# CederGroupHub/sparse-lm

Measured on AMD Instinct MI355X. Metric: fits/sec over 50-alpha Lasso path at n=100k p=5k, higher is better.
Workload: dtype f64

## Files before the change

sparse-lm_amd/csrc/ws_kernels.hpp:

```cpp
#pragma once
#include <type_traits>
#include <hip/hip_runtime.h>
#include <stdint.h>

#include "tail_kernels.hpp"
#include "newton_kernels.hpp"

namespace slm {

constexpr int WS_KCAP = 512;
constexpr int WS_KLDS = 112;
constexpr int WS_TILES = WS_KCAP / 16;
constexpr int WS_THREADS = 1024;
constexpr int WS_INNER_MAX = 400;
constexpr int WS_BB_ITERS = 14;
constexpr double WS_BB_MAX_STEP = 20.0;
constexpr double WS_INNER_TOL = 0.05;
constexpr int WS_MAX_REPEATS = 6;
constexpr int WS_NEWTON_AFTER = 16;
constexpr int WS_NEWTON_MAX = 256;
constexpr int WS_AFTER_DIRECT = 40;
constexpr double WS_NEWTON_RQ = 0.05;
constexpr int WS_NEWTON_REFUSALS = 4;
constexpr double WS_NEWTON_ENTER = 0.3;
constexpr int WS_NEWTON_RESOLVE = 5;
static_assert(NT_MAXT * NT_B == WS_KCAP, "the direct solve covers a full working set");

struct WsCtl {
  int32_t request;
  int32_t building;
  int32_t valid;
  int32_t K;
  int32_t Kreal;
  int32_t k_new;
  int32_t builds;
  int32_t appends;
  int32_t max_builds;
  int32_t disabled;
  int32_t misses;
  int32_t refined;
  int32_t counter;
  int32_t stale;
  int32_t overflows;
  int32_t sweep_new;
  int32_t sweep_miss;
  int32_t staged;
  int32_t inner_iters;
  int32_t hard;
  int32_t hard_next;
  int32_t newton_steps;
  int32_t newton_fails;
  int32_t newton_nopd;
  int32_t newton_trial[4];
  int32_t newton_ref[4];
  int32_t newton_factors;
  int32_t newton_unknowns;
  unsigned long long nt_ticks[SLM_MAX_LANES][6];
  int32_t nt_factors[SLM_MAX_LANES];
  unsigned long long solve_ticks[5];
  int32_t want_full[SLM_MAX_LANES];
  int32_t iters_hist[32];
  unsigned long long lane_ticks[SLM_MAX_LANES];
  int32_t last_point[SLM_MAX_LANES];
  int32_t repeats[SLM_MAX_LANES];
  int32_t last_cols[SLM_MAX_LANES];
  double Lw[SLM_MAX_LANES];
  int32_t carried;
  int32_t outgrown;
  int32_t served[SLM_MAX_LANES];
  int32_t hard_lane[SLM_MAX_LANES];
};

struct WsArgs {
  WsCtl* ws;
  int32_t* idx;
  int32_t* pos;
  int32_t* gs;
  int32_t* gl;
  double* score;
  double* XW;
  double* part;
  double* Gm;
  double* nt;
  double* Gx;
  const double* X;
  const double* XT;
  int64_t n, ld;
  const double* rw;
  int64_t rw_stride;
  double inv_n[SLM_MAX_LANES];
  int32_t set_of[SLM_MAX_LANES];
  int32_t set_lane[SLM_MAX_LANES];
  int32_t n_sets;
  int32_t nblk;
  const int32_t* owner;
  double theta;
  int32_t lookahead;
  int32_t append_max;
  int32_t k_init;
  int32_t bb_steps;
  int32_t one_solver;
  int32_t miss_factor;
  int32_t miss_div;
  double fill;
  int32_t power_iters;
  int32_t hard_call;
  int32_t keep_full;
};

constexpr int WS_HEAD_WORDS = 24;
static_assert(offsetof(WsCtl, hard_next) / 4 < WS_HEAD_WORDS, "the words the pass kernels decide on");
#define WS_HEAD(hd, field) ((hd)[offsetof(WsCtl, field) / 4])
__device__ __forceinline__ void ws_head_load(const WsCtl* ws, const int* gdone, int32_t* hd) {
  const int tid = threadIdx.x;
  if (tid < WS_HEAD_WORDS) hd[tid] = reinterpret_cast<const int32_t*>(ws)[tid];
  else if (tid == WS_HEAD_WORDS) hd[tid] = gdone ? gdone[0] : 0;
}

static __global__ void ws_ctl_init_kernel(WsCtl* ws, int max_builds) {
  if (threadIdx.x == 0) {
    ws->request = 1;
    ws->max_builds = max_builds;
  }
  if (threadIdx.x < SLM_MAX_LANES) ws->last_point[threadIdx.x] = -1;
}

struct BeginArgs {
  const PathCtl* h_ctl;
  PathCtl* ctl;
  const slm_path_point* h_pts;
  slm_path_point* pts;
  int64_t n_pts;
  int32_t* head;
  int32_t head_words;
  const double* lambda;
  double margin;
  double factor[SLM_MAX_LANES];
  WsCtl* ws;
  int32_t max_builds;
  int32_t n_lanes;
};
static __global__ __launch_bounds__(256) void solve_begin_kernel(SetupArgs s, BeginArgs b) {
  solve_setup_body(s);
  const int64_t stride = (int64_t)gridDim.x * blockDim.x;
  {
    static_assert(sizeof(slm_path_point) == 4 * sizeof(double), "points travel as doubles");
    const double* src = reinterpret_cast<const double*>(b.h_pts);
    double* dst = reinterpret_cast<double*>(b.pts);
    for (int64_t e = (int64_t)blockIdx.x * blockDim.x + threadIdx.x; e < 4 * b.n_pts; e += stride) dst[e] = src[e];
  }
  if (blockIdx.x != 0) return;
  for (int e = threadIdx.x; e < b.head_words; e += 256) b.head[e] = 0;
  {
    static_assert(sizeof(PathCtl) % sizeof(int32_t) == 0, "control blocks travel as words");
    const int32_t* src = reinterpret_cast<const int32_t*>(b.h_ctl);
    int32_t* dst = reinterpret_cast<int32_t*>(b.ctl);
    const int words = b.n_lanes * (int)(sizeof(PathCtl) / sizeof(int32_t));
    for (int e = threadIdx.x; e < words; e += 256) dst[e] = src[e];
  }
  __syncthreads();
  if (b.lambda != nullptr && (int)threadIdx.x < b.n_lanes && threadIdx.x < SLM_MAX_LANES) {
    const int l = threadIdx.x;
    double L0 = b.lambda[0] * b.margin;
    if (L0 <= 0.0) L0 = 1.0;
    const double L = L0 * b.factor[l];
    b.ctl[l].L = L;
    b.ctl[l].ak = 1.25 * L;
    b.ctl[l].Lhat = 0.5 * L0;
  }
  if (b.ws != nullptr) {
    if (threadIdx.x == 0) {
      b.ws->request = 1;
      b.ws->max_builds = b.max_builds;
    }
    if (threadIdx.x < SLM_MAX_LANES) b.ws->last_point[threadIdx.x] = -1;
  }
}

static __global__ __launch_bounds__(256) void ws_ctl_carry_kernel(WsCtl* ws, int max_builds) {
  __shared__ int keep_i[2];
  __shared__ double keep_L[SLM_MAX_LANES];
  if (threadIdx.x == 0) {
    keep_i[0] = ws->K;
    keep_i[1] = ws->Kreal;
  }
  if (threadIdx.x < SLM_MAX_LANES) keep_L[threadIdx.x] = ws->Lw[threadIdx.x];
  __syncthreads();
  int32_t* words = reinterpret_cast<int32_t*>(ws);
  for (int e = threadIdx.x; e < (int)(sizeof(WsCtl) / sizeof(int32_t)); e += 256) words[e] = 0;
  __syncthreads();
  if (threadIdx.x == 0) {
    ws->K = keep_i[0];
    ws->Kreal = keep_i[1];
    ws->valid = 1;
    ws->carried = 1;
    ws->max_builds = max_builds;
  }
  if (threadIdx.x < SLM_MAX_LANES) {
    ws->Lw[threadIdx.x] = keep_L[threadIdx.x];
    ws->last_point[threadIdx.x] = -1;
  }
}

__device__ __forceinline__ int block_excl_scan(int v, int* wave_tot , int* total) {
  const int lane = threadIdx.x & 63, wave = threadIdx.x >> 6;
  int inc = v;
#pragma unroll
  for (int off = 1; off < 64; off <<= 1) {
    const int t = __shfl_up(inc, off, 64);
    if (lane >= off) inc += t;
  }
  __syncthreads();
  if (lane == 63) wave_tot[wave] = inc;
  __syncthreads();
  int base = 0, tot = 0;
#pragma unroll
  for (int w = 0; w < TAIL_WAVES; ++w) {
    const int t = wave_tot[w];
    if (w < wave) base += t;
    tot += t;
  }
  *total = tot;
  return base + inc - v;
}

__device__ __forceinline__ void ws_score_body(TailArgs a, WsArgs w, const int chunk) {
  WsCtl* ws = w.ws;
  const int tid = threadIdx.x;
  __shared__ int32_t hd[WS_HEAD_WORDS + 1];
  __shared__ int lane_np[SLM_MAX_LANES];
  ws_head_load(ws, a.gdone, hd);
  if (tid < SLM_MAX_LANES) lane_np[tid] = tid < a.n_lanes ? a.ctl[tid].n_points : 0;
  __syncthreads();
  if (hd[WS_HEAD_WORDS] != 0 || WS_HEAD(hd, disabled)) return;
  const bool had_w = WS_HEAD(hd, valid) != 0;
  if (!WS_HEAD(hd, request) && !had_w) return;
  if (WS_HEAD(hd, builds) >= WS_HEAD(hd, max_builds) || WS_HEAD(hd, appends) >= 8 * WS_HEAD(hd, max_builds)) return;
  const bool singleton = a.singleton != 0;
  const int nitems = singleton ? a.p : a.G;
  __shared__ int lane_live[SLM_MAX_LANES];
  __shared__ double lane_sa[SLM_MAX_LANES], lane_sb[SLM_MAX_LANES];
  __shared__ int cnt[2];
  if (tid < SLM_MAX_LANES) {
    int live = 0;
    double sa = 0.0, sb = 0.0;
    if (tid < a.n_lanes) {
      const PathCtl* c = a.ctl + tid;
      live = !(c->done || c->idle);
      int path_end = 0;
      for (int l = 0; l < SLM_MAX_LANES; ++l) path_end = max(path_end, lane_np[l]);
      const int end = a.steal ? path_end : c->pt_off + c->n_points;
      int look = min(c->pt_off + c->point + max(w.lookahead, c->stride), end - 1);
      if (c->tail_pt >= 0 && c->point + c->stride >= c->n_points) look = c->pt_off + c->tail_pt;
      const slm_path_point pe = a.pts[look < 0 ? 0 : look];
      sa = pe.sa;
      sb = pe.sb;
    }
    lane_live[tid] = live;
    lane_sa[tid] = sa;
    lane_sb[tid] = sb;
  }
  if (tid == 0) cnt[0] = cnt[1] = 0;
  __syncthreads();

  const double inf = __builtin_huge_val();
  int n_new = 0, n_miss = 0;
  const int gt = chunk * (int)blockDim.x + tid;
  const int it = singleton ? gt : gt >> 4;
  if (singleton) {
    if (it < nitems) {
      double sc = 0.0;
      const int j = it;
      const bool in_w = had_w && w.pos[j] >= 0;
      for (int l0 = 0; l0 < a.n_lanes; l0 += 16) {
        double zp[16], zz[16], aa[16], bb[16], gg[16];
#pragma unroll
        for (int l = 0; l < 16; ++l) {
          const int ll = l0 + l < a.n_lanes ? l0 + l : 0;
          const int64_t off = (int64_t)ll * a.ld;
          zp[l] = a.zprev[off + j];
          zz[l] = a.z[off + j];
          aa[l] = a.a0[off + j];
          bb[l] = a.b0[off + j];
          gg[l] = a.g[(int64_t)ll * (a.ld + 16) + j];
        }
#pragma unroll
        for (int l = 0; l < 16; ++l) {
          if (l0 + l >= a.n_lanes || !lane_live[l0 + l]) continue;
          if (!in_w && had_w && zz[l] != zp[l]) n_miss += 1;
          if (zp[l] != 0.0) {
            sc = inf;
          } else {
            const double thr = lane_sa[l0 + l] * aa[l] + lane_sb[l0 + l] * bb[l];
            sc = fmax(sc, thr > 0.0 ? fabs(gg[l]) / thr : inf);
          }
        }
      }
      if (sc >= w.theta && !in_w) n_new += 1;
      w.score[it] = sc;
    }
  } else {
    static_assert(SLM_MAX_LANES % 16 == 0, "16-thread teams: a thread per (group, lane of a half)");
    const int l16 = tid & 15;
    const bool have = it < nitems;
// ... 190 lines not shown
            ws->stale = 1;
          }
          return;
        }
      }
      append = false;
      thr = w.theta;
    }
  }
  if (!append) {
    count_at(inf, false, &n_sel, nullptr);
    if (n_sel > (double)WS_KCAP) {
      if (tid == 0) {
        ws->overflows += 1;
        ws->outgrown += 1;
        if (had_w) {
          ws->request = 0;
          ws->stale = 1;
        } else {
          ws->request = 1;
          ws->valid = 0;
          if (ws->overflows >= 50) ws->disabled = 1;
        }
      }
      return;
    }
    const double nonzeros = n_sel;
    thr = fit_threshold(w.theta, false, fmax((double)w.k_init, nonzeros), &n_sel);
    for (int j = tid; j < p; j += WS_THREADS) w.pos[j] = -1;
  }
  for (int k = k_old * (append ? 1 : 0) + tid; k < WS_KCAP; k += WS_THREADS) {
    w.idx[k] = -1;
    w.gs[k] = k;
    w.gl[k] = 1;
  }
  __syncthreads();

  unsigned long long pick = 0ull;
  int mine = 0;
  if (cached) {
#pragma unroll
    for (int u = 0; u < 8; ++u) {
      if (c_sc[u] >= thr && !(append && c_inw[u])) {
        pick |= 1ull << u;
        mine += c_sz[u];
      }
    }
  } else {
    for (int it = i0; it < i1 && it - i0 < 64; ++it) {
      if (!(w.score[it] >= thr)) continue;
      if (append && w.pos[singleton ? it : a.order[a.gstart[it]]] >= 0) continue;
      pick |= 1ull << (it - i0);
      mine += singleton ? 1 : a.gstart[it + 1] - a.gstart[it];
    }
  }
  int total = 0;
  int at = (append ? k_old : 0) + block_excl_scan(mine, wave_tot, &total);
  __syncthreads();
  for (int it = i0; it < i1 && it - i0 < 64; ++it) {
    if (!((pick >> (it - i0)) & 1ull)) continue;
    if (singleton) {
      w.idx[at] = it;
      w.pos[it] = at;
      at += 1;
    } else {
      const int k0 = a.gstart[it], len = a.gstart[it + 1] - k0;
      for (int m = 0; m < len; ++m) {
        const int j = a.order[k0 + m];
        w.idx[at + m] = j;
        w.pos[j] = at + m;
        w.gs[at + m] = at;
        w.gl[at + m] = len;
      }
      at += len;
    }
  }
  if (tid == 0) {
    const int Kreal = (append ? k_old : 0) + total;
    ws->Kreal = Kreal;
    ws->K = max(16, (Kreal + 15) & ~15);
    ws->k_new = append ? k_old : 0;
    ws->building = 1;
    ws->valid = 0;
    ws->stale = 0;
    ws->counter = 0;
    if (append) {
      ws->appends += 1;
    } else {
      ws->builds += 1;
      for (int l = 0; l < SLM_MAX_LANES; ++l) ws->Lw[l] = 0.0;
    }
  }
}

static __global__ __launch_bounds__(WS_THREADS) void ws_select_kernel(TailArgs a, WsArgs w) { ws_select_body(a, w); }

static __global__ __launch_bounds__(256) void ws_gather_kernel(WsArgs w) {
  if (!w.ws->building) return;
  const int K = w.ws->K;
  const int k0 = w.ws->k_new + 32 * (int)blockIdx.y;
  if (k0 >= K) return;
  __shared__ double tile[32][33];
  const int tx = threadIdx.x & 31, ty = threadIdx.x >> 5;
  const int64_t row_tiles = (w.n + 31) / 32;
  int jcol[4];
#pragma unroll
  for (int u = 0; u < 4; ++u) {
    const int k = k0 + ty + 8 * u;
    jcol[u] = k < K ? w.idx[k] : -1;
  }
  for (int64_t rt = blockIdx.x; rt < row_tiles; rt += gridDim.x) {
    const int64_t i0 = rt * 32;
    const int64_t i = i0 + tx;
    double v[4];
#pragma unroll
    for (int u = 0; u < 4; ++u) {
      const int j = jcol[u];
      v[u] = (j >= 0 && i < w.n) ? (w.XT ? w.XT[((rt * w.ld + j) << 5) + tx] : w.X[i * w.ld + j]) : 0.0;
    }
    __syncthreads();
#pragma unroll
    for (int u = 0; u < 4; ++u) tile[ty + 8 * u][tx] = v[u];
    __syncthreads();
    for (int ii = ty; ii < 32; ii += 8) {
      const int64_t i = i0 + ii;
      const int k = k0 + tx;
      if (i < w.n && k < K) w.XW[i * WS_KCAP + k] = tile[tx][ii];
    }
  }
}

struct XtyArgs {
  const WsCtl* ws;
  const int32_t* idx;
  const double* XW;
  const double* y;
  double* part;
  double* g;
  double* gprev;
  double* z;
  PathCtl* ctl;
  const int* done;
  int64_t n, ld;
  double inv_n;
  int n_lanes, nblk;
};
static __global__ __launch_bounds__(512) void ws_xty_partial_kernel(XtyArgs a) {
  if (*a.done) return;
  __shared__ double red[8][WS_KCAP];
  __shared__ double red_yy[8];
  const int K = a.ws->K;
  const int lane = threadIdx.x & 63, wave = threadIdx.x >> 6;
  const int64_t rows = (a.n + gridDim.x - 1) / gridDim.x;
  const int64_t i0 = (int64_t)blockIdx.x * rows, i1 = i0 + rows < a.n ? i0 + rows : a.n;
  double acc[WS_KCAP / 64];
#pragma unroll
  for (int c = 0; c < WS_KCAP / 64; ++c) acc[c] = 0.0;
  double yy = 0.0;
  auto rows4 = [&](auto NC) {
    constexpr int C = decltype(NC)::value;
    for (int64_t i = i0 + wave; i < i1; i += 32) {
      double xv[4][C], yv[4];
#pragma unroll
      for (int r = 0; r < 4; ++r) {
        const bool in = i + 8 * r < i1;
        const int64_t ii = in ? i + 8 * r : i;
        yv[r] = in ? a.y[ii] : 0.0;
#pragma unroll
        for (int c = 0; c < C; ++c) {
          const int k = lane + 64 * c;
          xv[r][c] = a.XW[ii * WS_KCAP + (k < K ? k : 64 * c)];
        }
      }
#pragma unroll
      for (int r = 0; r < 4; ++r) {
        yy = __builtin_fma(yv[r], yv[r], yy);
#pragma unroll
        for (int c = 0; c < C; ++c) acc[c] = __builtin_fma(lane + 64 * c < K ? xv[r][c] : 0.0, yv[r], acc[c]);
      }
    }
  };
  switch ((K + 63) >> 6) {
    case 1: rows4(std::integral_constant<int, 1>{}); break;
    case 2: rows4(std::integral_constant<int, 2>{}); break;
    case 3: rows4(std::integral_constant<int, 3>{}); break;
    case 4: rows4(std::integral_constant<int, 4>{}); break;
    case 5: rows4(std::integral_constant<int, 5>{}); break;
    case 6: rows4(std::integral_constant<int, 6>{}); break;
    case 7: rows4(std::integral_constant<int, 7>{}); break;
    default: rows4(std::integral_constant<int, 8>{}); break;
  }
  static_assert(WS_KCAP / 64 == 8, "eight chunks of 64 positions");
#pragma unroll
  for (int c = 0; c < WS_KCAP / 64; ++c) red[wave][lane + 64 * c] = acc[c];
  if (lane == 0) red_yy[wave] = yy;
  __syncthreads();
  double* out = a.part + (int64_t)blockIdx.x * (WS_KCAP + 1);
  const int k = threadIdx.x;
  if (k < K) {
    double sum = 0.0;
#pragma unroll
    for (int w = 0; w < 8; ++w) sum += red[w][k];
    out[k] = sum;
  }
  if (k == WS_KCAP - 1) {
    double sum = 0.0;
#pragma unroll
    for (int w = 0; w < 8; ++w) sum += red_yy[w];
    out[WS_KCAP] = sum;
  }
}
static __global__ __launch_bounds__(512) void ws_xty_apply_kernel(XtyArgs a) {
  if (*a.done) return;
  __shared__ double red[4][128];
  __shared__ double ry[512];
  const int K = a.ws->K;
  const int kl = threadIdx.x & 127, q = threadIdx.x >> 7;
  const int k = (int)blockIdx.x * 128 + kl;
  if ((int)blockIdx.x * 128 >= K) return;
  double s[8] = {0, 0, 0, 0, 0, 0, 0, 0};
  if (k < K) {
    int b = q;
    for (; b + 28 < a.nblk; b += 32) {
#pragma unroll
      for (int u = 0; u < 8; ++u) s[u] += a.part[(int64_t)(b + 4 * u) * (WS_KCAP + 1) + k];
    }
    for (; b < a.nblk; b += 4) s[0] += a.part[(int64_t)b * (WS_KCAP + 1) + k];
  }
  red[q][kl] = ((s[0] + s[1]) + (s[2] + s[3])) + ((s[4] + s[5]) + (s[6] + s[7]));
  if (blockIdx.x == 0) ry[threadIdx.x] = (int)threadIdx.x < a.nblk ? a.part[(int64_t)threadIdx.x * (WS_KCAP + 1) + WS_KCAP] : 0.0;
  __syncthreads();
  if (q == 0 && k < K) {
    const int j = a.idx[k];
    if (j >= 0) {
      const double c = -((red[0][kl] + red[1][kl]) + (red[2][kl] + red[3][kl])) * a.inv_n;
      for (int l = 0; l < a.n_lanes; ++l) {
        a.g[(int64_t)l * (a.ld + 16) + j] = c;
        a.gprev[(int64_t)l * a.ld + j] = c;
        a.z[(int64_t)l * a.ld + j] = 0.0;
      }
    }
  }
  if (blockIdx.x == 0) {
    for (int off = 256; off >= 1; off >>= 1) {
      if ((int)threadIdx.x < off) ry[threadIdx.x] += ry[threadIdx.x + off];
      __syncthreads();
    }
    if (threadIdx.x < (unsigned)a.n_lanes) {
      const int l = threadIdx.x;
      const double loss0 = 0.5 * ry[0] * a.inv_n;
      a.g[(int64_t)l * (a.ld + 16) + a.ld] = loss0;
      a.ctl[l].hist[0] = loss0;
      a.ctl[l].loss_base = loss0;
    }
  }
}

static __global__ __launch_bounds__(256) void ws_block_owner_kernel(const double* rw, int64_t rw_stride, WsArgs w, int32_t* owner) {
  __shared__ int cls[SLM_MAX_LANES];
  __shared__ int red[2][4];
  const int tid = threadIdx.x;
  const int64_t b = blockIdx.x;
  const int64_t base = w.n / w.nblk, rem = w.n % w.nblk;
  const int64_t r0 = b * base + (b < rem ? b : rem);
  const int64_t nrows = base + (b < rem ? 1 : 0);
  for (int st = 0; st < w.n_sets; ++st) {
    const double* v = rw + (int64_t)w.set_lane[st] * rw_stride + r0;
    int zeros = 1, ones = 1;
    for (int64_t i = tid; i < nrows; i += 256) {
      const double x = v[i];
      zeros &= (x == 0.0);
      ones &= (x == 1.0);
    }
    zeros = __all(zeros);
    ones = __all(ones);
    if ((tid & 63) == 0) {
      red[0][tid >> 6] = zeros;
      red[1][tid >> 6] = ones;
    }
    __syncthreads();
    if (tid == 0) {
      const int z = red[0][0] & red[0][1] & red[0][2] & red[0][3], o = red[1][0] & red[1][1] & red[1][2] & red[1][3];
      cls[st] = z ? 0 : (o ? 1 : 2);
    }
    __syncthreads();
  }
  if (tid == 0) {
    int first_ones = -1;
    for (int st = 0; st < w.n_sets; ++st) {
      int o = st;
      if (cls[st] == 0) o = -1;
      else if (cls[st] == 1) {
        if (first_ones < 0) first_ones = st;
        o = first_ones;
      }
      owner[(int64_t)st * w.nblk + b] = o;
    }
  }
}

typedef double ws_d4 __attribute__((ext_vector_type(4)));
constexpr int WS_GRAM_THREADS = 512;
constexpr int WS_GRAM_ZCHUNKS = 4;

static __global__ __launch_bounds__(WS_GRAM_THREADS) void ws_gram_kernel(WsArgs w) {
  if (!w.ws->building) return;
  __shared__ ws_d4 comb[2][16][64];
  const int K = w.ws->K;
  const int tile_lo = w.ws->k_new >> 4;
  const int tid = threadIdx.x, lane = tid & 63;
  const int wave = __builtin_amdgcn_readfirstlane(tid >> 6);
  const int tiles = K >> 4;
  const bool row_split = (tile_lo > 0 || tiles <= 8) && tiles - tile_lo <= 4 * WS_GRAM_ZCHUNKS;
  const int set = blockIdx.y;
  const int64_t b = blockIdx.x;
  if (w.owner != nullptr && w.owner[(int64_t)set * w.nblk + b] != set) return;
  const int64_t base = w.n / w.nblk, rem = w.n % w.nblk;
  const int64_t r0 = b * base + (b < rem ? b : rem);
  const int64_t nrows = base + (b < rem ? 1 : 0);
  const double* rw = w.rw ? w.rw + (int64_t)w.set_lane[set] * w.rw_stride : nullptr;
  const int part = row_split ? (wave >> 1) : 0;
  const int64_t steps = (nrows + 3) >> 2;
  const int64_t s_begin = row_split ? 4 * (steps * part / 4) : 0;
  const int64_t s_end = row_split ? min(nrows, 4 * (steps * (part + 1) / 4)) : nrows;

  for (int slice = 0; slice < 4 * WS_GRAM_ZCHUNKS; ++slice) {
  const int zhi = slice >> 2;
  if (8 * (slice & 3) >= tiles) continue;
  if (row_split ? (tile_lo + 4 * zhi >= tiles) : (zhi >= 2)) continue;
  const int wj = 2 * (slice & 3) + (wave & 1);
  const int ntj = min(4, max(0, tiles - 4 * wj));
  const int ibase = row_split ? tile_lo + 4 * zhi : 4 * (4 * zhi + (wave >> 1));
  const int ti_lo = row_split ? 0 : max(0, tile_lo - ibase);
  const int nti = min(4, max(0, tiles - ibase));
  const bool active = ti_lo < nti && ntj > 0;
  if (!row_split && !active) continue;
  ws_d4 acc[4][4];
#pragma unroll
  for (int ti = 0; ti < 4; ++ti)
#pragma unroll
    for (int tj = 0; tj < 4; ++tj) acc[ti][tj] = ws_d4{0.0, 0.0, 0.0, 0.0};

  const int kk = lane >> 4, c = lane & 15;
  if (active) {
    const int ta_max = WS_TILES - 1;
    const double* rwp = rw ? rw : w.XW;
    const bool has_rw = rw != nullptr;
    auto load = [&](int64_t s, double(&av)[4], double(&bv)[4], double& wgt) {
      const int64_t i = s + kk;
      const bool ok = i < s_end;
      const int64_t row = r0 + (ok ? i : 0);
      const double wv = rwp[has_rw ? row : 0];
      const double* xr = w.XW + row * WS_KCAP + c;
#pragma unroll
      for (int t = 0; t < 4; ++t) {
        av[t] = xr[16 * min(ibase + t, ta_max)];
        bv[t] = xr[16 * min(4 * wj + t, ta_max)];
      }
      wgt = ok ? (has_rw ? wv : 1.0) : 0.0;
    };
    auto mma = [&](const double(&av)[4], const double(&bv)[4], double wgt) {
#pragma unroll
      for (int ti = 0; ti < 4; ++ti) {
        if (ti >= ti_lo && ti < nti) {
          const double a = av[ti] * wgt;
#pragma unroll
          for (int tj = 0; tj < 4; ++tj)
            if (tj < ntj) acc[ti][tj] = __builtin_amdgcn_mfma_f64_16x16x4f64(a, bv[tj], acc[ti][tj], 0, 0, 0);
        }
      }
    };
    double a0[4], b0[4], a1[4], b1[4], a2[4], b2[4], a3[4], b3[4], w0, w1, w2, w3;
    load(s_begin, a0, b0, w0);
    load(s_begin + 4, a1, b1, w1);
    load(s_begin + 8, a2, b2, w2);
    for (int64_t s = s_begin; s < s_end; s += 16) {
      load(s + 12, a3, b3, w3);
      mma(a0, b0, w0);
      load(s + 16, a0, b0, w0);
      mma(a1, b1, w1);
      load(s + 20, a1, b1, w1);
      mma(a2, b2, w2);
      load(s + 24, a2, b2, w2);
      mma(a3, b3, w3);
    }
  }
  if (row_split) {
    for (int round = 0; round < 4; ++round) {
      if (part == round && active) {
#pragma unroll
        for (int ti = 0; ti < 4; ++ti)
#pragma unroll
          for (int tj = 0; tj < 4; ++tj) {
            if (ti < nti && tj < ntj) {
              if (round > 0) acc[ti][tj] += comb[wave & 1][ti * 4 + tj][lane];
              if (round < 3) comb[wave & 1][ti * 4 + tj][lane] = acc[ti][tj];
            }
          }
      }
      __syncthreads();
    }
  }
  if (!row_split || (part == 3 && active)) {
#pragma unroll
  for (int ti = 0; ti < 4; ++ti) {
    if (ti < ti_lo || ti >= nti) continue;
#pragma unroll
    for (int tj = 0; tj < 4; ++tj) {
      if (tj >= ntj) continue;
      const int64_t tile = (int64_t)(ibase + ti) * WS_TILES + (4 * wj + tj);
      double* out = w.part + (((int64_t)set * (WS_TILES * WS_TILES) + tile) * w.nblk + b) * 256;
#pragma unroll
      for (int r = 0; r < 4; ++r) out[(kk + 4 * r) * 16 + c] = acc[ti][tj][r];
    }
  }
  }
  if (row_split) __syncthreads();
  }
}

static __global__ __launch_bounds__(256) void ws_gram_reduce_kernel(WsArgs w) {
  WsCtl* ws = w.ws;
  if (!ws->building) return;
  const int K = ws->K;
  const int row_lo = (ws->k_new >> 4) << 4;
  const int set = blockIdx.y;
  const int tile = blockIdx.x, I = tile / WS_TILES, J = tile % WS_TILES;
  const int tiles = K >> 4, I_lo = row_lo >> 4;
  if (I < I_lo || I >= tiles || J >= tiles) return;
  const int i = 16 * I + (threadIdx.x >> 4), j = 16 * J + (threadIdx.x & 15);
  {
    const double* src = w.part + (((int64_t)set * (WS_TILES * WS_TILES) + tile) * w.nblk) * 256 + threadIdx.x;
    double s4[4] = {0.0, 0.0, 0.0, 0.0};
    int b = 0;
    if (w.owner != nullptr) {
      __shared__ int64_t off_s[512];
      static_assert(sizeof(off_s) >= 8 * 512, "nblk <= 512");
      for (int bb = threadIdx.x; bb < w.nblk; bb += 256) {
        const int o = w.owner[(int64_t)set * w.nblk + bb];
        off_s[bb] = o < 0 ? -1 : (int64_t)(o - set) * (WS_TILES * WS_TILES) * w.nblk * 256;
      }
      __syncthreads();
      for (; b + 32 <= w.nblk; b += 32) {
        double v[32];
#pragma unroll
        for (int u = 0; u < 32; ++u) {
          const int64_t o = off_s[b + u];
          v[u] = o == -1 ? 0.0 : src[(int64_t)(b + u) * 256 + o];
        }
#pragma unroll
        for (int u = 0; u < 32; ++u) s4[u & 3] += v[u];
      }
      for (; b < w.nblk; ++b) {
        const int64_t o = off_s[b];
        s4[b & 3] += o == -1 ? 0.0 : src[(int64_t)b * 256 + o];
      }
    }
    for (; b + 32 <= w.nblk; b += 32) {
      double v[32];
#pragma unroll
      for (int u = 0; u < 32; ++u) v[u] = src[(int64_t)(b + u) * 256];
#pragma unroll
      for (int u = 0; u < 32; ++u) s4[u & 3] += v[u];
    }
    for (; b < w.nblk; ++b) s4[b & 3] += src[(int64_t)b * 256];
    double s = ((s4[0] + s4[1]) + (s4[2] + s4[3])) * w.inv_n[set];
    double* Gs = (w.Gx ? w.Gx : w.Gm) + (int64_t)set * (WS_KCAP * WS_KCAP);
    Gs[i * WS_KCAP + j] = s;
    if (j < row_lo) Gs[j * WS_KCAP + i] = s;
  }
  __threadfence();
  __syncthreads();
  if (threadIdx.x == 0) {
    const int total = (tiles - I_lo) * tiles * (int)gridDim.y;
    if (atomicAdd(&ws->counter, 1) + 1 == total) {
      ws->counter = 0;
      if (w.Gx) {
        ws->staged = 1;
      } else {
        ws->request = 0;
        ws->valid = 1;
        __threadfence();
        ws->building = 0;
      }
    }
  }
}

constexpr int WS_PUBLISH_BLOCKS = 64;
static __global__ __launch_bounds__(256) void ws_publish_kernel(WsArgs w) {
  WsCtl* ws = w.ws;
  if (!ws->building || !ws->staged) return;
  const int K = ws->K;
  const int row_lo = (ws->k_new >> 4) << 4;
  const int set = blockIdx.y;
  for (int i = blockIdx.x; i < K; i += gridDim.x)
    for (int j = threadIdx.x; j < K; j += 256)
      if (i >= row_lo || j >= row_lo) {
        const int64_t at = (int64_t)set * (WS_KCAP * WS_KCAP) + (int64_t)i * WS_KCAP + j;
        w.Gm[at] = w.Gx[at];
      }
  __threadfence();
  __syncthreads();
  if (threadIdx.x == 0) {
    const int total = gridDim.x * gridDim.y;
    if (atomicAdd(&ws->counter, 1) + 1 == total) {
      ws->counter = 0;
      ws->staged = 0;
      ws->request = 0;
      ws->valid = 1;
      __threadfence();
      ws->building = 0;
    }
  }
}

template <int NV>
__device__ __forceinline__ void ws_sum(double (&v)[NV], double (*lds)[TAIL_WAVES], int nwc) {
  const int lane = threadIdx.x & 63;
  const int wave = __builtin_amdgcn_readfirstlane(threadIdx.x >> 6);
  if (wave < nwc) {
#pragma unroll
    for (int k = 0; k < NV; ++k) v[k] = wave_sum_lane63(v[k]);
  }
  __syncthreads();
  if (wave < nwc && lane == 63) {
#pragma unroll
    for (int k = 0; k < NV; ++k) lds[k][wave] = v[k];
  }
  __syncthreads();
  if (nwc == 4) {
#pragma unroll
    for (int k = 0; k < NV; ++k) v[k] = group_sum_all<4>(lds[k][lane & 3]);
  } else {
#pragma unroll
    for (int k = 0; k < NV; ++k) v[k] = group_sum_all<8>(lds[k][lane & 7]);
  }
}

struct WsSolveLds {
  double delta[WS_KCAP];
  double uim[WS_KCAP];
  double part[WS_THREADS];
  double Gl[WS_KLDS * WS_KLDS];
  NtShared nts;
  double nv[WS_KCAP];
  double xsl[WS_KCAP];
  double rgl[WS_KCAP];
  double pbl[WS_KCAP];
  double scale2;
  int nz[WS_KCAP];
  int act[WS_KCAP];
  int rank_of[WS_KCAP];
  int nnz, m;
};

template <bool GROUPED, bool DIRECT>
__device__ __forceinline__ bool ws_refine_lane(TailArgs a, const WsArgs& w, double (*red)[TAIL_WAVES], WsSolveLds& sh) {
  double (&delta)[WS_KCAP] = sh.delta;
  double (&uim)[WS_KCAP] = sh.uim;
  int (&nz)[WS_KCAP] = sh.nz;
  int& nnz_s = sh.nnz;
  double (&part)[WS_THREADS] = sh.part;
  double (&Gl)[WS_KLDS * WS_KLDS] = sh.Gl;
  NtShared& nts = sh.nts;
  double (&nv)[WS_KCAP] = sh.nv;
  int (&act)[WS_KCAP] = sh.act;
  int (&rank_of)[WS_KCAP] = sh.rank_of;
  int& m_s = sh.m;
  double (&xsl)[WS_KCAP] = sh.xsl;
  double (&rgl)[WS_KCAP] = sh.rgl;
  double (&pbl)[WS_KCAP] = sh.pbl;
  double& scale2_s = sh.scale2;
  const int lane_id = blockIdx.x;
  PathCtl* ctl = a.ctl + lane_id;
  WsCtl* ws = w.ws;
  if (!ws->valid || ws->building || ws->disabled) return true;
  const int tid = threadIdx.x;
  const int p = a.p;
  const int K = __builtin_amdgcn_readfirstlane(ws->K);
  const int set = w.set_of[lane_id];
  const double* Gm = w.Gm + (int64_t)set * (WS_KCAP * WS_KCAP);
  {
    const int64_t off = (int64_t)lane_id * a.ld;
    a.beta += off; a.z += off; a.zprev += off; a.gprev += off;
    a.a0 += off; a.b0 += off; a.d0 += off;
    a.pts += ctl->pt_off;
  }
  if (ws->stale) {
    double out[1] = {0.0};
    for (int j = tid; j < p; j += WS_THREADS)
      if (w.pos[j] < 0 && a.z[j] != a.zprev[j]) out[0] += 1.0;
    block_sum<1>(out, red);
    if (out[0] != 0.0) return true;
  }
  const int point_now = ctl->point + ctl->pt_off;
  const int reps = (ws->last_point[lane_id] == point_now && ws->last_cols[lane_id] == ws->Kreal) ? ws->repeats[lane_id] : 0;
  if (reps >= WS_MAX_REPEATS) return true;
  const int hard_now = w.hard_call ? ws->hard : ws->hard_lane[lane_id];
  if (!DIRECT && w.nt != nullptr && hard_now != 0) {
    if (tid == 0) ws->want_full[lane_id] = 1;
    return false;
  }

  unsigned long long tk_s = wall_clock64();
  auto mark = [&](int slot) {
    if (tid == 0 && lane_id == 0) {
      const unsigned long long now = wall_clock64();
      ws->solve_ticks[slot] += now - tk_s;
      tk_s = now;
    }
  };
  const slm_path_point pt = a.pts[ctl->point];
  const int mode = ctl->mode;
  const double tol = ctl->tol;
  const bool group_pen = (pt.sb != 0.0) || (pt.sd != 0.0);
  const bool g_lds = K <= WS_KLDS;
  if (g_lds) {
    for (int e = tid; e < K * K; e += WS_THREADS) {
      const int r = e / K, c = e - r * K;
      Gl[e] = Gm[r * WS_KCAP + c];
    }
  }

  const int tsh = K <= 256 ? 2 : 1;
  const int TPC = 1 << tsh;
  const int KP = WS_THREADS >> tsh;
  const int k = tid & (KP - 1), q = tid >> (10 - tsh);
  static_assert(WS_THREADS == 1024, "q = tid >> (10 - tsh)");
  const int nwc = KP >> 6;
  const int j = k < K ? w.idx[k] : -1;
  const bool live = j >= 0;
  const bool mine = live && q == 0;
  const int jj = live ? j : 0;
  const double z0 = live ? a.zprev[jj] : 0.0;
  const double g0 = live ? a.gprev[jj] : 0.0;
  const double x_start = live ? a.z[jj] : 0.0;
  const double pa = live ? pt.sa * a.a0[jj] : 0.0;
  const int gsk = live ? w.gs[k] : 0, glk = live ? w.gl[k] : 1;
  const int gix = a.singleton ? jj : a.gid[jj];
  const double pb = live ? pt.sb * a.b0[gix] : 0.0;
  const double pd = live ? pt.sd * a.d0[gix] : 0.0;
  __syncthreads();

  auto matvec = [&](double val, bool dense) -> double {
    if (q == 0) delta[k] = (k < K) ? val - z0 : 0.0;
    __syncthreads();
    double acc = 0.0;
    if (g_lds) {
      if (k < K) {
#pragma unroll 4
        for (int c = q; c < K; c += TPC) acc = __builtin_fma(Gl[c * K + k], delta[c], acc);
      }
    } else if (dense) {
      if (k < K) {
        for (int c = __builtin_amdgcn_readfirstlane(q); c < K; c += 16 * TPC) {
          double gv[16];
#pragma unroll
          for (int u = 0; u < 16; ++u) gv[u] = Gm[(c + u * TPC < K ? c + u * TPC : c) * WS_KCAP + k];
#pragma unroll
          for (int u = 0; u < 16; ++u) acc = __builtin_fma(gv[u], c + u * TPC < K ? delta[c + u * TPC] : 0.0, acc);
        }
      }
    } else {
      if (tid < 64) {
        int basep = 0;
        for (int c0 = 0; c0 < K; c0 += 64) {
          const int kk = c0 + tid;
          const bool nzq = kk < K && delta[kk] != 0.0;
          const uint64_t m = __ballot(nzq);
          if (nzq) nz[basep + __popcll(m & ((1ull << tid) - 1ull))] = kk;
          basep += __popcll(m);
        }
        if (tid == 0) nnz_s = basep;
      }
      __syncthreads();
      const int nnz = __builtin_amdgcn_readfirstlane(nnz_s);
      const int qs = __builtin_amdgcn_readfirstlane(q);
      if (k < K) {
        for (int m = qs; m < nnz; m += 12 * TPC) {
          int cc[12];
          double gv[12];
#pragma unroll
          for (int u = 0; u < 12; ++u) cc[u] = __builtin_amdgcn_readfirstlane(nz[m + u * TPC < nnz ? m + u * TPC : m]);
#pragma unroll
          for (int u = 0; u < 12; ++u) gv[u] = Gm[cc[u] * WS_KCAP + k];
#pragma unroll
          for (int u = 0; u < 12; ++u) acc = __builtin_fma(gv[u], m + u * TPC < nnz ? delta[cc[u]] : 0.0, acc);
        }
      }
    }
    part[tid] = acc;
    __syncthreads();
    double tot = part[k];
    for (int qq = 1; qq < TPC; ++qq) tot += part[qq * KP + k];
    return tot;
  };
  auto prox_w = [&](double v, double s) -> double {
    double u = live ? soft(v, s * pa) : 0.0;
    if (group_pen) {
      if (a.singleton) {
        const double nrm = fabs(u);
        const double sc = nrm > 0.0 ? fmax(0.0, 1.0 - s * pb / nrm) : 0.0;
        u *= sc / (1.0 + s * pd);
      } else {
        __syncthreads();
        if (q == 0) uim[k] = u;
        __syncthreads();
        double ss = 0.0;
        for (int m = 0; m < glk; ++m) {
          const double t = uim[gsk + m];
          ss = __builtin_fma(t, t, ss);
        }
        const double nrm = sqrt(ss);
        const double sc = (nrm > 0.0 ? fmax(0.0, 1.0 - s * pb / nrm) : 0.0) / (1.0 + s * pd);
        u *= sc;
      }
    }
    return u;
  };
  auto pen_part = [&](double val) -> double {
    double pv = 0.0;
    if (mine) {
      pv = pa * fabs(val);
      if (group_pen && a.singleton) pv += pb * fabs(val) + 0.5 * pd * val * val;
    }
    if (group_pen && !a.singleton) {
      __syncthreads();
      if (q == 0) uim[k] = live ? val : 0.0;
      __syncthreads();
      if (mine && gsk == k) {
        double ss = 0.0;
        for (int m = 0; m < glk; ++m) ss = __builtin_fma(uim[k + m], uim[k + m], ss);
        pv += pb * sqrt(ss) + 0.5 * pd * ss;
      }
    }
    return pv;
  };

  mark(0);
  double Lw = ws->Lw[set];
  if (!(Lw > 0.0)) {
    double vec = (k < K) ? 1.0 + 0.37 * (double)(((k * 2654435761u) >> 24) & 0xffu) / 255.0 : 0.0;
    double lam = 0.0;
    for (int itp = 0; itp < w.power_iters; ++itp) {
      const double y = matvec(vec + z0, true);
      double s[1] = {q == 0 && k < K ? y * y : 0.0};
      ws_sum<1>(s, red, nwc);
      lam = sqrt(s[0]);
      vec = lam > 0.0 ? y / lam : 0.0;
    }
    Lw = lam * 1.1;
    if (!(Lw > 0.0)) return true;
  }

  constexpr bool group_face = GROUPED;
  const bool newton_capable = w.nt != nullptr;
  double* ntF = newton_capable ? w.nt + (int64_t)lane_id * NT_SCRATCH : nullptr;
  double* ntD = newton_capable ? ntF + (int64_t)NT_TILES * 256 : nullptr;
  auto block_min = [&](double val) -> double {
#pragma unroll
    for (int off = 32; off >= 1; off >>= 1) val = fmin(val, __shfl_xor(val, off, 64));
    __syncthreads();
    if ((tid & 63) == 0) red[0][tid >> 6] = val;
    __syncthreads();
    double mm = red[0][0];
#pragma unroll
    for (int wv = 1; wv < TAIL_WAVES; ++wv) mm = fmin(mm, red[0][wv]);
    return mm;
  };
  int resolve_cap = WS_NEWTON_RESOLVE;
  auto direct_step = [&](double& x, double Lmax, double* mu_out, bool want_mu) -> int {
   if constexpr (GROUPED) {
    return 0;
   } else {
    *mu_out = 0.0;
    const double thr = pa + pb;
// ... 741 lines not shown
```

Baseline: 16930.

## Compute only lower-triangular Gram tiles and mirror them in reduce

The Gram kernel now computes only the tiles with J <= I, using a bitmask of needed slots per wave. When the working set is small (at most 7 tiles, no incremental rows) it uses a packed triangular mapping so both waves share the tile columns, with compile-time unrolled MFMA selection. The reduce kernel skips upper tiles, writes each diagonal entry once and mirrors the off-diagonal ones. This cuts redundant MFMA work and partial-sum traffic roughly in half, at the cost of more complex indexing and a changed completion-counter formula that must match the launched tiles.

Result: no change. 16840 (-0.5%).

```diff
diff --git a/sparse-lm_amd/csrc/ws_kernels.hpp b/sparse-lm_amd/csrc/ws_kernels.hpp
--- a/sparse-lm_amd/csrc/ws_kernels.hpp
+++ b/sparse-lm_amd/csrc/ws_kernels.hpp
@@ -1,5 +1,6 @@
 #pragma once
 #include <type_traits>
+#include <utility>
 #include <hip/hip_runtime.h>
 #include <stdint.h>
 
@@ -796,6 +797,19 @@
 typedef double ws_d4 __attribute__((ext_vector_type(4)));
 constexpr int WS_GRAM_THREADS = 512;
 constexpr int WS_GRAM_ZCHUNKS = 4;
+constexpr int WS_GRAM_TRI_TILES = 7;
+
+constexpr int ws_tri_row(int t) {
+  int i = 0;
+  while ((i + 1) * (i + 2) / 2 <= t) ++i;
+  return i;
+}
+constexpr int ws_tri_col(int t) { return t - ws_tri_row(t) * (ws_tri_row(t) + 1) / 2; }
+
+template <int... Ks, class F>
+__device__ __forceinline__ void ws_unrolled(std::integer_sequence<int, Ks...>, F&& f) {
+  (f(std::integral_constant<int, Ks>{}), ...);
+}
 
 static __global__ __launch_bounds__(WS_GRAM_THREADS) void ws_gram_kernel(WsArgs w) {
   if (!w.ws->building) return;
@@ -806,6 +820,9 @@
   const int wave = __builtin_amdgcn_readfirstlane(tid >> 6);
   const int tiles = K >> 4;
   const bool row_split = (tile_lo > 0 || tiles <= 8) && tiles - tile_lo <= 4 * WS_GRAM_ZCHUNKS;
+  const bool tri = tile_lo == 0 && tiles <= WS_GRAM_TRI_TILES;
+  const int h = wave & 1;
+  const int col_walks = (tiles + 7) >> 3;
   const int set = blockIdx.y;
   const int64_t b = blockIdx.x;
   if (w.owner != nullptr && w.owner[(int64_t)set * w.nblk + b] != set) return;
@@ -817,26 +834,38 @@
   const int64_t steps = (nrows + 3) >> 2;
   const int64_t s_begin = row_split ? 4 * (steps * part / 4) : 0;
   const int64_t s_end = row_split ? min(nrows, 4 * (steps * (part + 1) / 4)) : nrows;
+  const int kk = lane >> 4, c = lane & 15;
 
   for (int slice = 0; slice < 4 * WS_GRAM_ZCHUNKS; ++slice) {
-  const int zhi = slice >> 2;
-  if (8 * (slice & 3) >= tiles) continue;
-  if (row_split ? (tile_lo + 4 * zhi >= tiles) : (zhi >= 2)) continue;
-  const int wj = 2 * (slice & 3) + (wave & 1);
-  const int ntj = min(4, max(0, tiles - 4 * wj));
-  const int ibase = row_split ? tile_lo + 4 * zhi : 4 * (4 * zhi + (wave >> 1));
-  const int ti_lo = row_split ? 0 : max(0, tile_lo - ibase);
-  const int nti = min(4, max(0, tiles - ibase));
-  const bool active = ti_lo < nti && ntj > 0;
-  if (!row_split && !active) continue;
-  ws_d4 acc[4][4];
-#pragma unroll
-  for (int ti = 0; ti < 4; ++ti)
-#pragma unroll
-    for (int tj = 0; tj < 4; ++tj) acc[ti][tj] = ws_d4{0.0, 0.0, 0.0, 0.0};
-
-  const int kk = lane >> 4, c = lane & 15;
-  if (active) {
+  const int zhi = slice >> 2, q = slice & 3;
+  if (q >= col_walks) continue;
+  if (tri ? (slice > 0) : row_split ? (tile_lo + 4 * zhi >= tiles) : (zhi >= 2)) continue;
+  const int abase = tri ? 0 : row_split ? tile_lo + 4 * zhi : 4 * (4 * zhi + (wave >> 1));
+  const int bbase = tri ? 4 : row_split ? 2 * q + h : 4 * (2 * q + h);
+  const int bstep = (!tri && row_split) ? 2 * col_walks : 1;
+  auto slot_tile = [&](int k, int& I, int& J) -> bool {
+    if (tri) {
+      I = ws_tri_row(2 * k + h);
+      J = ws_tri_col(2 * k + h);
+      return I < tiles;
+    }
+    I = abase + (k >> 2);
+    J = bbase + bstep * (k & 3);
+    return I >= tile_lo && I < tiles && J <= I;
+  };
+  unsigned need = 0;
+#pragma unroll
+  for (int k = 0; k < 16; ++k) {
+    int I, J;
+    if (slot_tile(k, I, J)) need |= 1u << k;
+  }
+  need = __builtin_amdgcn_readfirstlane(need);
+  if (!row_split && need == 0) continue;
+  ws_d4 acc[16];
+#pragma unroll
+  for (int k = 0; k < 16; ++k) acc[k] = ws_d4{0.0, 0.0, 0.0, 0.0};
+
+  if (need != 0) {
     const int ta_max = WS_TILES - 1;
     const double* rwp = rw ? rw : w.XW;
     const bool has_rw = rw != nullptr;
@@ -848,65 +877,79 @@
       const double* xr = w.XW + row * WS_KCAP + c;
 #pragma unroll
       for (int t = 0; t < 4; ++t) {
-        av[t] = xr[16 * min(ibase + t, ta_max)];
-        bv[t] = xr[16 * min(4 * wj + t, ta_max)];
+        av[t] = xr[16 * min(abase + t, ta_max)];
+        bv[t] = xr[16 * min(bbase + bstep * t, ta_max)];
       }
       wgt = ok ? (has_rw ? wv : 1.0) : 0.0;
     };
     auto mma = [&](const double(&av)[4], const double(&bv)[4], double wgt) {
 #pragma unroll
       for (int ti = 0; ti < 4; ++ti) {
-        if (ti >= ti_lo && ti < nti) {
+        if ((need >> (4 * ti)) & 15u) {
           const double a = av[ti] * wgt;
 #pragma unroll
           for (int tj = 0; tj < 4; ++tj)
-            if (tj < ntj) acc[ti][tj] = __builtin_amdgcn_mfma_f64_16x16x4f64(a, bv[tj], acc[ti][tj], 0, 0, 0);
+            if ((need >> (4 * ti + tj)) & 1u)
+              acc[4 * ti + tj] = __builtin_amdgcn_mfma_f64_16x16x4f64(a, bv[tj], acc[4 * ti + tj], 0, 0, 0);
         }
       }
     };
-    double a0[4], b0[4], a1[4], b1[4], a2[4], b2[4], a3[4], b3[4], w0, w1, w2, w3;
-    load(s_begin, a0, b0, w0);
-    load(s_begin + 4, a1, b1, w1);
-    load(s_begin + 8, a2, b2, w2);
-    for (int64_t s = s_begin; s < s_end; s += 16) {
-      load(s + 12, a3, b3, w3);
-      mma(a0, b0, w0);
-      load(s + 16, a0, b0, w0);
-      mma(a1, b1, w1);
-      load(s + 20, a1, b1, w1);
-      mma(a2, b2, w2);
-      load(s + 24, a2, b2, w2);
-      mma(a3, b3, w3);
-    }
+    auto mma_tri = [&](auto hc) {
+      return [&](const double(&av)[4], const double(&bv)[4], double wgt) {
+        const double cv[8] = {av[0], av[1], av[2], av[3], bv[0], bv[1], bv[2], bv[3]};
+        double cw[WS_GRAM_TRI_TILES];
+#pragma unroll
+        for (int t = 0; t < WS_GRAM_TRI_TILES; ++t) cw[t] = cv[t] * wgt;
+        ws_unrolled(std::make_integer_sequence<int, WS_GRAM_TRI_TILES * (WS_GRAM_TRI_TILES + 1) / 4>{}, [&](auto kc) {
+          constexpr int k = decltype(kc)::value, t = 2 * k + decltype(hc)::value;
+          constexpr int I = ws_tri_row(t), J = ws_tri_col(t);
+          if ((need >> k) & 1u) acc[k] = __builtin_amdgcn_mfma_f64_16x16x4f64(cw[I], cv[J], acc[k], 0, 0, 0);
+        });
+      };
+    };
+    auto walk = [&](auto&& mm) {
+      double a0[4], b0[4], a1[4], b1[4], a2[4], b2[4], a3[4], b3[4], w0, w1, w2, w3;
+      load(s_begin, a0, b0, w0);
+      load(s_begin + 4, a1, b1, w1);
+      load(s_begin + 8, a2, b2, w2);
+      for (int64_t s = s_begin; s < s_end; s += 16) {
+        load(s + 12, a3, b3, w3);
+        mm(a0, b0, w0);
+        load(s + 16, a0, b0, w0);
+        mm(a1, b1, w1);
+        load(s + 20, a1, b1, w1);
+        mm(a2, b2, w2);
+        load(s + 24, a2, b2, w2);
+        mm(a3, b3, w3);
+      }
+    };
+    if (!tri) walk(mma);
+    else if (h == 0) walk(mma_tri(std::integral_constant<int, 0>{}));
+    else walk(mma_tri(std::integral_constant<int, 1>{}));
   }
   if (row_split) {
     for (int round = 0; round < 4; ++round) {
-      if (part == round && active) {
-#pragma unroll
-        for (int ti = 0; ti < 4; ++ti)
-#pragma unroll
-          for (int tj = 0; tj < 4; ++tj) {
-            if (ti < nti && tj < ntj) {
-              if (round > 0) acc[ti][tj] += comb[wave & 1][ti * 4 + tj][lane];
-              if (round < 3) comb[wave & 1][ti * 4 + tj][lane] = acc[ti][tj];
-            }
+      if (part == round && need != 0) {
+#pragma unroll
+        for (int k = 0; k < 16; ++k) {
+          if ((need >> k) & 1u) {
+            if (round > 0) acc[k] += comb[h][k][lane];
+            if (round < 3) comb[h][k][lane] = acc[k];
           }
+        }
       }
       __syncthreads();
     }
   }
-  if (!row_split || (part == 3 && active)) {
-#pragma unroll
-  for (int ti = 0; ti < 4; ++ti) {
-    if (ti < ti_lo || ti >= nti) continue;
-#pragma unroll
-    for (int tj = 0; tj < 4; ++tj) {
-      if (tj >= ntj) continue;
-      const int64_t tile = (int64_t)(ibase + ti) * WS_TILES + (4 * wj + tj);
-      double* out = w.part + (((int64_t)set * (WS_TILES * WS_TILES) + tile) * w.nblk + b) * 256;
-#pragma unroll
-      for (int r = 0; r < 4; ++r) out[(kk + 4 * r) * 16 + c] = acc[ti][tj][r];
-    }
+  if (!row_split || part == 3) {
+#pragma unroll
+  for (int k = 0; k < 16; ++k) {
+    int I, J;
+    if (!slot_tile(k, I, J)) continue;
+    const int64_t tile = (int64_t)I * WS_TILES + J;
+    double* out = w.part + (((int64_t)set * (WS_TILES * WS_TILES) + tile) * w.nblk + b) * 256;
+#pragma unroll
+    for (int r = 0; r < 4; ++r) out[(kk + 4 * r) * 16 + c] = acc[k][r];
   }
   }
   if (row_split) __syncthreads();
@@ -921,7 +964,7 @@
   const int set = blockIdx.y;
   const int tile = blockIdx.x, I = tile / WS_TILES, J = tile % WS_TILES;
   const int tiles = K >> 4, I_lo = row_lo >> 4;
-  if (I < I_lo || I >= tiles || J >= tiles) return;
+  if (I < I_lo || I >= tiles || J > I) return;
   const int i = 16 * I + (threadIdx.x >> 4), j = 16 * J + (threadIdx.x & 15);
   {
     const double* src = w.part + (((int64_t)set * (WS_TILES * WS_TILES) + tile) * w.nblk) * 256 + threadIdx.x;
@@ -960,13 +1003,15 @@
     for (; b < w.nblk; ++b) s4[b & 3] += src[(int64_t)b * 256];
     double s = ((s4[0] + s4[1]) + (s4[2] + s4[3])) * w.inv_n[set];
     double* Gs = (w.Gx ? w.Gx : w.Gm) + (int64_t)set * (WS_KCAP * WS_KCAP);
-    Gs[i * WS_KCAP + j] = s;
-    if (j < row_lo) Gs[j * WS_KCAP + i] = s;
+    if (j <= i) {
+      Gs[i * WS_KCAP + j] = s;
+      if (j < i) Gs[j * WS_KCAP + i] = s;
+    }
   }
   __threadfence();
   __syncthreads();
   if (threadIdx.x == 0) {
-    const int total = (tiles - I_lo) * tiles * (int)gridDim.y;
+    const int total = (tiles * (tiles + 1) - I_lo * (I_lo + 1)) / 2 * (int)gridDim.y;
     if (atomicAdd(&ws->counter, 1) + 1 == total) {
       ws->counter = 0;
       if (w.Gx) {
```
